# tj12323/GeoPurify

Measured on AMD Instinct MI355X. Metric: scenes/sec (ScanNet-val shape) + pooled-feature GB/s vs HBM peak, higher is better.
Workload: dtype f32 (student convolutions and pooling: f16 hi/lo split operands, 3 MFMAs per product, fp32 accumulate)

## Files before the change

geopurify_amd/csrc/sparse_conv_v2.hip:

```cpp
#include <cstring>
#include <type_traits>
#include <rocprim/device/device_scan.hpp>

#include <hip/hip_fp16.h>

#include <stdlib.h>

#include "gp_common.h"
#include "gp_gfx950.h"

namespace {

constexpr int TM = 256, TN = 256, TK = 32;
constexpr int NT2 = 512;
constexpr int APITCH = 32;
__device__ __forceinline__ int sw_slot(int row, int slot) {
    const int h = (0x78 >> (((row >> 2) & 3) * 2)) & 3;
    return slot ^ h;
}

__device__ __forceinline__ void pair_decode(int64_t i, int kv, const int32_t *__restrict__ R, int nchunks, int &c, int &k, int64_t &u) {
    const int row_q = (int)(i / kv);
    int lo = 0, hi = nchunks - 1;
    while (lo < hi) {
// ... 658 lines not shown
        continue;
    }
    for (int c = lane * 4; c < cout; c += 256) {
        float4 a = conv_gather_sum<GS_NL>(P, mypos, kv, cout, c, pair_base);
        float4 sc = scale ? *reinterpret_cast<const float4 *>(scale + c) : make_float4(1.f, 1.f, 1.f, 1.f);
        float4 sh = shift ? *reinterpret_cast<const float4 *>(shift + c) : make_float4(0.f, 0.f, 0.f, 0.f);
        a.x = a.x * sc.x + sh.x; a.y = a.y * sc.y + sh.y; a.z = a.z * sc.z + sh.z; a.w = a.w * sc.w + sh.w;
        if (residual) {
            float4 r = *reinterpret_cast<const float4 *>(residual + u * ld_res + c);
            a.x += r.x; a.y += r.y; a.z += r.z; a.w += r.w;
        }
        if (res_hi) {
            const _Float16 *rph = r_il ? res_hi + u * ld_rh + ((c >> 5) << 6) + (c & 31) : res_hi + u * ld_rh + c;
                    const _Float16 *rpl = r_il ? rph + 32 : res_lo + u * ld_rh + c;
                    const f16x4 rh = *reinterpret_cast<const f16x4 *>(rph), rl = *reinterpret_cast<const f16x4 *>(rpl);
            const float ri = res_inv ? res_inv[u] : 1.f;
            a.x += ((float)rh[0] + (float)rl[0]) * ri; a.y += ((float)rh[1] + (float)rl[1]) * ri;
            a.z += ((float)rh[2] + (float)rl[2]) * ri; a.w += ((float)rh[3] + (float)rl[3]) * ri;
        }
        if (relu) { a.x = fmaxf(a.x, 0.f); a.y = fmaxf(a.y, 0.f); a.z = fmaxf(a.z, 0.f); a.w = fmaxf(a.w, 0.f); }
        if (y) *reinterpret_cast<float4 *>(y + u * ld_y + c) = a;
        if (y_hi) {
            float v[4] = {a.x, a.y, a.z, a.w};
            f16x4 h, l;
            gp_split_f16<4>(v, h, l);
            _Float16 *ph = y_il ? y_hi + u * ld_yh + ((c >> 5) << 6) + (c & 31) : y_hi + u * ld_yh + c;
            _Float16 *pl = y_il ? ph + 32 : y_lo + u * ld_yh + c;
            *reinterpret_cast<f16x4 *>(ph) = h;
            *reinterpret_cast<f16x4 *>(pl) = l;
        }
    }
    }
}

template <int NL>
__device__ __forceinline__ void conv_gather_sum_q24(const unsigned char *__restrict__ pb, int64_t e_off, int mypos, int kv,
                                                    int cout, int c, bool act, int pair_base, float (&a)[8]) {
#pragma unroll
    for (int j = 0; j < 8; ++j) a[j] = 0.f;
    unsigned long long m = __ballot(mypos >= 0) & ((kv >= 64) ? ~0ull : ((1ull << kv) - 1ull));
    const int nq = cout >> 7;
    const unsigned char *pb_e = pb + e_off;
    while (m) {
        int kk[NL];
        u32x4 th[NL];
        u32x2 tl[NL];
        unsigned te[NL];
        int cntv = 0;
#pragma unroll
        for (int i = 0; i < NL; ++i) {
            if (m) { kk[i] = __builtin_ctzll(m); m &= m - 1; ++cntv; } else kk[i] = -1;
        }
#pragma unroll
        for (int i = 0; i < NL; ++i)
            if (i < cntv) {
                const unsigned pos = (unsigned)(__shfl(mypos, kk[i], 64) - pair_base);
                if (act) {
                    const unsigned o = (pos * (unsigned)cout + ((unsigned)c & ~127u)) * 3u, f = ((unsigned)c >> 3) & 15u;
                    th[i] = *reinterpret_cast<const u32x4 *>(pb + o + f * 16u);
                    tl[i] = *reinterpret_cast<const u32x2 *>(pb + o + 256u + f * 8u);
                    te[i] = pb_e[pos * (unsigned)nq + ((unsigned)c >> 7)];
                }
            }
#pragma unroll
        for (int i = 0; i < NL; ++i)
            if (i < cntv && act) {
                const float s = te[i] == 255u ? __uint_as_float(0x7fc00000u) : __uint_as_float((te[i] - 21u) << 23);
                const unsigned d[6] = {th[i][0], th[i][1], th[i][2], th[i][3], tl[i][0], tl[i][1]};
#pragma unroll
                for (int g = 0; g < 2; ++g) {
                    const unsigned u0 = __builtin_amdgcn_perm(0u, d[g * 3], 0x0c020100u);
                    const unsigned u1 = __builtin_amdgcn_perm(d[g * 3 + 1], d[g * 3], 0x0c050403u);
                    const unsigned u2 = __builtin_amdgcn_perm(d[g * 3 + 2], d[g * 3 + 1], 0x0c040302u);
                    const unsigned u3 = __builtin_amdgcn_perm(0u, d[g * 3 + 2], 0x0c030201u);
                    a[g * 4 + 0] = fmaf((float)u0 - 4194304.f, s, a[g * 4 + 0]);
                    a[g * 4 + 1] = fmaf((float)u1 - 4194304.f, s, a[g * 4 + 1]);
                    a[g * 4 + 2] = fmaf((float)u2 - 4194304.f, s, a[g * 4 + 2]);
                    a[g * 4 + 3] = fmaf((float)u3 - 4194304.f, s, a[g * 4 + 3]);
                }
            }
    }
}

template <bool WIDE , bool NO_CENTRE = false >
__global__ void __launch_bounds__(256) __attribute__((amdgpu_waves_per_eu(4, 4)))
conv_phase2_q24_kernel(const unsigned char *__restrict__ pb, int64_t e_off, const int32_t *__restrict__ pair_pos, int64_t nv,
                       int kv, int cout, const float *__restrict__ scale, const float *__restrict__ shift,
                       const float *__restrict__ residual, int64_t ld_res, int relu, float *__restrict__ y, int64_t ld_y,
                       _Float16 *__restrict__ y_hi, _Float16 *__restrict__ y_lo, int64_t ld_yh, int64_t row_begin, int64_t row_count,
                       int pair_base, float *__restrict__ y_inv_scale, const _Float16 *__restrict__ res_hi,
                       const _Float16 *__restrict__ res_lo, int64_t ld_rh, const float *__restrict__ res_inv, int plane_flags) {
    const bool y_il = (plane_flags & 2) != 0, r_il = (plane_flags & 4) != 0;
    const int lane = gp_lane();
    const int64_t wave0 = (blockIdx.x * (int64_t)blockDim.x + threadIdx.x) >> 6, n_waves = ((int64_t)gridDim.x * blockDim.x) >> 6;
    const int64_t row_end = (row_begin + row_count < nv) ? row_begin + row_count : nv;
    int64_t u = row_begin + wave0;
    if (u >= row_end) return;
    const bool rowscale = y_inv_scale && y_hi && cout <= 1024;
    const int kv_read = NO_CENTRE ? (kv >> 1) : -1;
    int mypos_next = (lane < kv && lane != kv_read) ? pair_pos[(int64_t)lane * nv + u] : -1;
    float sc0[8], sh0[8];
    {
        const int c = lane * 8;
#pragma unroll
        for (int h = 0; h < 2; ++h) {
            const float4 a = (scale && c < cout) ? *reinterpret_cast<const float4 *>(scale + c + h * 4) : make_float4(1.f, 1.f, 1.f, 1.f);
            const float4 b = (shift && c < cout) ? *reinterpret_cast<const float4 *>(shift + c + h * 4) : make_float4(0.f, 0.f, 0.f, 0.f);
            sc0[h * 4] = a.x; sc0[h * 4 + 1] = a.y; sc0[h * 4 + 2] = a.z; sc0[h * 4 + 3] = a.w;
            sh0[h * 4] = b.x; sh0[h * 4 + 1] = b.y; sh0[h * 4 + 2] = b.z; sh0[h * 4 + 3] = b.w;
        }
    }
    for (; u < row_end; u += n_waves) {
        const int mypos = mypos_next;
        if (u + n_waves < row_end) mypos_next = (lane < kv && lane != kv_read) ? pair_pos[(int64_t)lane * nv + u + n_waves] : -1;
        float av[WIDE ? 2 : 1][8];
        float amax = 0.f;
        auto block = [&](int c0, float (&a)[8]) {
            const int c = c0 + lane * 8;
            const bool act = c < cout;
            conv_gather_sum_q24<WIDE ? 4 : GS_NL>(pb, e_off, mypos, kv, cout, c, act, pair_base, a);
            if (!act) return;
            if (c0 == 0) {
#pragma unroll
                for (int j = 0; j < 8; ++j) a[j] = a[j] * sc0[j] + sh0[j];
            } else {
                float scv[8], shv[8];
#pragma unroll
                for (int h = 0; h < 2; ++h) {
                    const float4 sc = scale ? *reinterpret_cast<const float4 *>(scale + c + h * 4) : make_float4(1.f, 1.f, 1.f, 1.f);
                    const float4 sh = shift ? *reinterpret_cast<const float4 *>(shift + c + h * 4) : make_float4(0.f, 0.f, 0.f, 0.f);
                    scv[h * 4] = sc.x; scv[h * 4 + 1] = sc.y; scv[h * 4 + 2] = sc.z; scv[h * 4 + 3] = sc.w;
                    shv[h * 4] = sh.x; shv[h * 4 + 1] = sh.y; shv[h * 4 + 2] = sh.z; shv[h * 4 + 3] = sh.w;
                }
#pragma unroll
                for (int j = 0; j < 8; ++j) a[j] = a[j] * scv[j] + shv[j];
            }
            if (residual) {
                const float4 r0 = *reinterpret_cast<const float4 *>(residual + u * ld_res + c);
                const float4 r1 = *reinterpret_cast<const float4 *>(residual + u * ld_res + c + 4);
                a[0] += r0.x; a[1] += r0.y; a[2] += r0.z; a[3] += r0.w; a[4] += r1.x; a[5] += r1.y; a[6] += r1.z; a[7] += r1.w;
            }
            if (res_hi) {
                const _Float16 *rph = r_il ? res_hi + u * ld_rh + ((c >> 5) << 6) + (c & 31) : res_hi + u * ld_rh + c;
                const _Float16 *rpl = r_il ? rph + 32 : res_lo + u * ld_rh + c;
                const f16x8 rh = *reinterpret_cast<const f16x8 *>(rph), rl = *reinterpret_cast<const f16x8 *>(rpl);
                const float ri = res_inv ? res_inv[u] : 1.f;
#pragma unroll
                for (int j = 0; j < 8; ++j) a[j] += ((float)rh[j] + (float)rl[j]) * ri;
            }
            if (relu) {
#pragma unroll
                for (int j = 0; j < 8; ++j) a[j] = fmaxf(a[j], 0.f);
            }
            if (y) {
                *reinterpret_cast<float4 *>(y + u * ld_y + c) = make_float4(a[0], a[1], a[2], a[3]);
                *reinterpret_cast<float4 *>(y + u * ld_y + c + 4) = make_float4(a[4], a[5], a[6], a[7]);
            }
#pragma unroll
            for (int j = 0; j < 8; ++j) amax = fmaxf(amax, fabsf(a[j]));
        };
        auto split_store = [&](int c0, const float (&a)[8], float s) {
            const int c = c0 + lane * 8;
            if (c >= cout) return;
            f16x8 h, l;
#pragma unroll
            for (int j = 0; j < 8; ++j) gp_split_f16(a[j] * s, h, l, j);
            _Float16 *ph = y_il ? y_hi + u * ld_yh + ((c >> 5) << 6) + (c & 31) : y_hi + u * ld_yh + c;
            _Float16 *pl = y_il ? ph + 32 : y_lo + u * ld_yh + c;
            *reinterpret_cast<f16x8 *>(ph) = h;
            *reinterpret_cast<f16x8 *>(pl) = l;
        };
        block(0, av[0]);
        if (!rowscale && y_hi) split_store(0, av[0], 1.f);
        if constexpr (WIDE) {
            block(512, av[1]);
            if (!rowscale && y_hi) split_store(512, av[1], 1.f);
        }
        if (rowscale) {
            amax = gp_wave_max(amax);
            const float s = gp_pow2_for(amax);
            if (lane == 0) y_inv_scale[u] = 1.f / s;
            split_store(0, av[0], s);
            if constexpr (WIDE) split_store(512, av[1], s);
        } else if constexpr (WIDE) {
            for (int c0 = 1024; c0 < cout; c0 += 512) {
                block(c0, av[0]);
                if (y_hi) split_store(c0, av[0], 1.f);
            }
        }
    }
}

__global__ void split_rows_scaled_kernel(const float *__restrict__ x, int64_t ld_x, int d, int64_t n, _Float16 *__restrict__ hi,
// ... 151 lines not shown

extern "C" size_t gp_conv_chunk_plan_workspace_bytes(int64_t nv, int32_t granule_rows) {
    if (nv <= 0 || granule_rows <= 0) return 0;
    return (size_t)((nv + granule_rows - 1) / granule_rows) * 32 * sizeof(int32_t);
}
extern "C" int gp_conv_chunk_plan(const int32_t *nbr_map, int64_t nv, int32_t kv, int32_t granule_rows, int32_t col_tiles,
                                  int32_t target_tiles, int32_t max_chunks, int32_t *chunk_row_off, int32_t *n_chunks, void *workspace,
                                  size_t workspace_bytes, void *stream_) {
    GP_CHECK_ARG(nbr_map && chunk_row_off && n_chunks && workspace && nv > 0 && kv > 0 && kv <= 32, "gp_conv_chunk_plan: null/empty argument");
    GP_CHECK_ARG(granule_rows >= 64 && granule_rows <= 65535 && col_tiles >= 1 && target_tiles >= col_tiles && max_chunks >= 1, "gp_conv_chunk_plan: bad sizes");
    const int64_t ngran = (nv + granule_rows - 1) / granule_rows;
    GP_CHECK_ARG(workspace_bytes >= gp_conv_chunk_plan_workspace_bytes(nv, granule_rows), "gp_conv_chunk_plan: workspace too small");
    hipStream_t s = gp_stream(stream_);
    int32_t *cnt = static_cast<int32_t *>(workspace);
    chunk_count_kernel<<<dim3((unsigned)ngran, (unsigned)kv), 256, 0, s>>>(nbr_map, nv, kv, granule_rows, cnt);
    chunk_plan_kernel<<<1, 256, 0, s>>>(cnt, (int)ngran, kv, granule_rows, nv, col_tiles, target_tiles, max_chunks, chunk_row_off, n_chunks);
    GP_CHECK_LAUNCH();
    return GP_OK;
}

extern "C" int gp_conv_weights_split(const float *w, int32_t kv, int32_t cin, int32_t cout, float scale_pow2,
                                     void *w_hi, void *w_lo, void *stream_) {
    GP_CHECK_ARG(w && w_hi && w_lo && kv > 0 && cin > 0 && cout > 0, "gp_conv_weights_split: null/empty argument");
    weight_split_kernel<<<2048, 256, 0, gp_stream(stream_)>>>(w, kv, cin, cout, scale_pow2, static_cast<_Float16 *>(w_hi),
                                                              static_cast<_Float16 *>(w_lo));
    GP_CHECK_LAUNCH();
    return GP_OK;
}

extern "C" int gp_conv_weights_split_blocked(const float *w, int32_t kv, int32_t cin, int32_t cout, float scale_pow2, void *w_hi,
                                             void *w_lo, int32_t transpose_flip, void *stream_) {
    GP_CHECK_ARG(w && w_hi && w_lo && kv > 0 && cin > 0 && cout > 0, "gp_conv_weights_split_blocked: null/empty argument");
    GP_CHECK_ARG(cin % TK == 0 && cout % TN == 0, "gp_conv_weights_split_blocked: cin=%d must be a multiple of %d and cout=%d of %d", cin, TK, cout, TN);
    GP_CHECK_ARG(!transpose_flip || ((reinterpret_cast<uintptr_t>(w) & 15) == 0), "gp_conv_weights_split_blocked: w must be 16-byte aligned");
    weight_split_blocked_kernel<<<(unsigned)((int64_t)kv * (cout / TN) * (cin / TK)), 256, 0, gp_stream(stream_)>>>(
        w, kv, cin, cout, scale_pow2, static_cast<_Float16 *>(w_hi), static_cast<_Float16 *>(w_lo), transpose_flip);
    GP_CHECK_LAUNCH();
    return GP_OK;
}

extern "C" int gp_split_f16(const float *x, int64_t ld_x, int32_t d, int64_t n, void *hi, void *lo, int64_t ld_h,
                            void *stream_) {
    GP_CHECK_ARG(x && hi && lo && n > 0 && d > 0 && d % 4 == 0 && ld_x % 4 == 0 && ld_h % 4 == 0, "gp_split_f16: bad argument");
    split_rows_kernel<<<2048, 256, 0, gp_stream(stream_)>>>(x, ld_x, d, n, static_cast<_Float16 *>(hi), static_cast<_Float16 *>(lo), ld_h);
    GP_CHECK_LAUNCH();
    return GP_OK;
}

extern "C" int gp_pow2_scale(const float *x, int64_t ld_x, int32_t d, int64_t n, float *scale2, void *workspace,
                             size_t workspace_bytes, void *stream_) {
    GP_CHECK_ARG(x && scale2 && workspace && workspace_bytes >= 4 && n > 0 && d > 0 && d % 4 == 0 && ld_x % 4 == 0,
                 "gp_pow2_scale: bad argument");
    hipStream_t s = gp_stream(stream_);
    GP_CHECK_HIP(hipMemsetAsync(workspace, 0, 4, s));
    amax_kernel<<<1024, 256, 0, s>>>(x, ld_x, d, n, static_cast<unsigned *>(workspace));
    pow2_scale_kernel<<<1, 1, 0, s>>>(static_cast<const unsigned *>(workspace), scale2);
    GP_CHECK_LAUNCH();
    return GP_OK;
}

extern "C" int gp_split_f16_scaled(const float *x, int64_t ld_x, int32_t d, int64_t n, void *hi, void *lo, int64_t ld_h,
                                   const float *scale, float *row_inv_scale, const int32_t *dst_row, void *stream_) {
    GP_CHECK_ARG(x && hi && n > 0 && d > 0 && d % 4 == 0 && ld_x % 4 == 0 && ld_h % 4 == 0, "gp_split_f16_scaled: bad argument");
    GP_CHECK_ARG(lo || (d % 32 == 0 && ld_h >= 2 * (int64_t)d), "gp_split_f16_scaled: lo = NULL asks for interleaved rows in hi: d %% 32 == 0 and ld_h >= 2 d");
    GP_CHECK_ARG(!(scale && row_inv_scale), "gp_split_f16_scaled: one global scale OR per-row scales");
    int64_t waves = n < 16384 ? n : 16384;
    split_rows_scaled_kernel<<<(unsigned)((waves * 64 + 255) / 256), 256, 0, gp_stream(stream_)>>>(
        x, ld_x, d, n, static_cast<_Float16 *>(hi), static_cast<_Float16 *>(lo), ld_h, scale, row_inv_scale, dst_row);
    GP_CHECK_LAUNCH();
    return GP_OK;
}

extern "C" int gp_sparse_conv_f16x3(const float *x, int64_t ld_x, const void *x_hi, const void *x_lo, int64_t ld_xh,
                                    const int32_t *pair_in, const int32_t *pair_pos,
                                    const int32_t *pair_off, const int32_t *tile_start, const int32_t *tile_desc,
                                    int32_t nseg, int64_t num_pairs, int64_t nv, int32_t kv,
                                    const void *w_hi, const void *w_lo, int32_t cin, int32_t cout, float *partial,
                                    const float *scale, const float *shift, const float *residual, int64_t ld_res,
                                    int32_t relu, float *y, int64_t ld_y, void *y_hi, void *y_lo, int64_t ld_yh,
                                    int32_t num_chunks, const int32_t *chunk_row_off_host, const int32_t *chunk_tile_off_host,
                                    const int32_t *chunk_pair_off_host, const float *x_row_inv_scale, float *y_row_inv_scale,
                                    const void *res_hi, const void *res_lo, int64_t ld_rh, const float *res_row_inv_scale, int32_t w_blocked,
                                    int32_t plane_flags, void *stream_) {
    GP_CHECK_ARG(plane_flags >= 0 && plane_flags < 32, "gp_sparse_conv_f16x3: plane_flags is a mask of 1 (x interleaved), 2 (y interleaved), 4 (residual interleaved), 8 (fp32 partial rows), 16 (one dense offset: phase 1 writes y)");
    const bool direct = (plane_flags & 16) != 0;
    GP_CHECK_ARG(!direct || (kv == 1 && num_pairs == nv && x_hi && y && ld_y == cout && !scale && !shift && !residual && !res_hi && !relu && !y_hi &&
                             !y_row_inv_scale && !(g_gp_knobs[3] & 16)),
                 "gp_sparse_conv_f16x3: plane_flags bit 4 is for kv = 1 with a pair for every row, pre-split x, contiguous fp32 y and no epilogue");
    GP_CHECK_ARG(!(plane_flags & 1) || (x_hi && ld_xh % 64 == 0 && cin % 32 == 0), "gp_sparse_conv_f16x3: interleaved x rows come as ONE tensor (x_hi) of 2 x cin halfs per row");
    GP_CHECK_ARG(!(plane_flags & 2) || (y_hi && ld_yh % 64 == 0 && (uintptr_t)y_hi % 16 == 0), "gp_sparse_conv_f16x3: interleaved y rows go to ONE tensor (y_hi) of 2 x cout halfs per row");
    GP_CHECK_ARG(!(plane_flags & 4) || (res_hi && ld_rh % 64 == 0), "gp_sparse_conv_f16x3: interleaved residual rows come as ONE tensor (res_hi)");
    GP_CHECK_ARG(w_blocked == 0 || w_blocked == 1, "gp_sparse_conv_f16x3: w_blocked is 0 (row-major weights) or 1 (gp_conv_weights_split_blocked)");
    GP_CHECK_ARG(!res_hi || ((res_lo || (plane_flags & 4)) && !residual && ld_rh % 8 == 0 && (uintptr_t)res_hi % 16 == 0 && (uintptr_t)res_lo % 16 == 0),
                 "gp_sparse_conv_f16x3: the residual comes as fp32 rows OR as 16-byte aligned split planes (res_hi + res_lo), not both");
    GP_CHECK_ARG(res_hi || (!res_lo && !res_row_inv_scale), "gp_sparse_conv_f16x3: res_lo / res_row_inv_scale belong to res_hi");
    GP_CHECK_ARG((x || (x_hi && (x_lo || (plane_flags & 1)))) && pair_in && pair_pos && pair_off && tile_start && tile_desc && nseg > 0 && w_hi && w_lo && partial && (y || y_hi), "gp_sparse_conv_f16x3: null argument");
    GP_CHECK_ARG(!x_hi || (ld_xh % 8 == 0 && (uintptr_t)x_hi % 16 == 0 && (uintptr_t)x_lo % 16 == 0), "gp_sparse_conv_f16x3: pre-split rows must be 16-byte aligned");
    GP_CHECK_ARG(!(plane_flags & 1) || !(g_gp_knobs[3] & 16), "gp_sparse_conv_f16x3: interleaved x rows need the LDS-DMA path");
    GP_CHECK_ARG(!y_hi || ((y_lo || (plane_flags & 2)) && ld_yh % 4 == 0), "gp_sparse_conv_f16x3: y_hi/y_lo come as a pair");
    GP_CHECK_ARG(!x_row_inv_scale || x_hi, "gp_sparse_conv_f16x3: x_row_inv_scale belongs to pre-split operands (x_hi/x_lo)");
    GP_CHECK_ARG(!y_row_inv_scale || (y_hi && cout <= 1024), "gp_sparse_conv_f16x3: y_row_inv_scale needs y_hi/y_lo and cout <= 1024");
    GP_CHECK_ARG(nv > 0 && num_pairs > 0 && (kv == 27 || kv == 1), "gp_sparse_conv_f16x3: bad sizes");
    GP_CHECK_ARG(cin % TK == 0, "gp_sparse_conv_f16x3: cin=%d must be a multiple of %d", cin, TK);
    GP_CHECK_ARG(x_hi || (ld_x % 4 == 0 && (uintptr_t)x % 16 == 0), "gp_sparse_conv_f16x3: x rows must be 16-byte aligned");
    GP_SMEM_ATTR(conv_phase1_kernel<false>, sizeof(V2Smem));
    GP_SMEM_ATTR(conv_phase1_kernel<true>, sizeof(V2Smem));
    constexpr size_t P1_DMA_SMEM = sizeof(V2Smem) + TM * sizeof(float);
    GP_SMEM_ATTR(conv_phase1_dma_kernel, P1_DMA_SMEM);
    GP_SMEM_ATTR(conv_phase1_tuning_kernel, P1_DMA_SMEM);
    GP_SMEM_ATTR(conv_phase1_stamp_kernel, P1_DMA_SMEM);

    uint64_t *stamp = static_cast<uint64_t *>(g_gp_debug_ptr[1]);
    GP_CHECK_ARG(cout % TN == 0, "gp_sparse_conv_f16x3: cout=%d must be a multiple of %d on this path", cout, TN);
    hipStream_t s = gp_stream(stream_);
    int n_tiles = cout / TN;
    GP_CHECK_ARG((num_chunks >= 1) == (chunk_tile_off_host != nullptr) && (num_chunks >= 1) == (chunk_pair_off_host != nullptr) &&
                     (num_chunks >= 1) == (chunk_row_off_host != nullptr),
                 "gp_sparse_conv_f16x3: num_chunks=%d needs ALL THREE host chunk tables (row, tile and pair offsets), num_chunks=0 needs none",
                 num_chunks);
    if (num_chunks >= 1) {
        bool rows_ok = chunk_row_off_host[0] == 0 && chunk_row_off_host[num_chunks] == nv;
        for (int c = 0; c < num_chunks && rows_ok; ++c) rows_ok = chunk_row_off_host[c + 1] > chunk_row_off_host[c];
        GP_CHECK_ARG(rows_ok, "gp_sparse_conv_f16x3: the %d chunk row offsets do not cover rows 0 .. %lld in ascending order", num_chunks, (long long)nv);
    }
    const bool chunked = num_chunks >= 1;
    const int nchunk = chunked ? num_chunks : 1;
    constexpr int p2_wg_per_cu = 6;
    bool q24_fits = !(plane_flags & 8);
    for (int c = 0; c < nchunk; ++c) {
        const int64_t cp = chunked ? (int64_t)chunk_pair_off_host[c + 1] - chunk_pair_off_host[c] : num_pairs;
        if (cp * cout * 3 + 32 >= ((int64_t)1 << 32)) q24_fits = false;
    }
    for (int c = 0; c < nchunk; ++c) {
        int tile_begin = chunked ? chunk_tile_off_host[c] : 0;
        int tile_count = chunked ? chunk_tile_off_host[c + 1] - tile_begin : (int)(num_pairs / TM + nseg);
        int pair_base = chunked ? chunk_pair_off_host[c] : 0;
        int64_t row_begin = chunked ? chunk_row_off_host[c] : 0;
        int64_t row_count = chunked ? chunk_row_off_host[c + 1] - row_begin : nv;
        const int64_t chunk_pairs = chunked ? (int64_t)chunk_pair_off_host[c + 1] - pair_base : num_pairs;
        const int64_t q_e_off = (chunk_pairs * cout * 3 + 15) & ~(int64_t)15;
        const bool dma_path = x_hi && !(g_conv_ablate & 16);
        const bool q24 = dma_path && !(g_conv_ablate & 32) && q24_fits;
        if (tile_count > 0) {
            int64_t nblocks = (((int64_t)tile_count * n_tiles + 7) / 8) * 8;
            const int tune = (g_conv_ablate & ~16) | ((dma_path && (!q24_fits || direct)) ? 32 : 0);
#define P1_ARGS static_cast<const _Float16 *>(x_hi), static_cast<const _Float16 *>(x_lo), ld_xh, pair_in, pair_off, tile_start,              \
                reinterpret_cast<const int4 *>(tile_desc), nseg, kv, static_cast<const _Float16 *>(w_hi), static_cast<const _Float16 *>(w_lo), \
                cin, cout, direct ? y + (int64_t)pair_base * cout : partial, n_tiles, tune, tile_begin, tile_count, pair_base, x_row_inv_scale, stamp, \
                q_e_off, w_blocked, plane_flags & 1
            if (dma_path) {
                GP_CHECK_ARG(!stamp || g_gp_debug_bytes[1] >= (size_t)nblocks * 16 * sizeof(uint64_t),
                             "gp_sparse_conv_f16x3: the stamp buffer of gp_debug_ptr(1) holds %zu bytes, this launch writes %zu",
                             g_gp_debug_bytes[1], (size_t)nblocks * 16 * sizeof(uint64_t));
                if (stamp) conv_phase1_stamp_kernel<<<(unsigned)nblocks, NT2, P1_DMA_SMEM, s>>>(P1_ARGS);
                else if (tune) conv_phase1_tuning_kernel<<<(unsigned)nblocks, NT2, P1_DMA_SMEM, s>>>(P1_ARGS);
                else conv_phase1_dma_kernel<<<(unsigned)nblocks, NT2, P1_DMA_SMEM, s>>>(P1_ARGS);
            } else {
                GP_CHECK_ARG(x, "gp_sparse_conv_f16x3: fp32 x required for the register-staged path");
                GP_CHECK_ARG(!x_row_inv_scale, "gp_sparse_conv_f16x3: the register-staged path splits unscaled fp32 rows");
#define P1R_ARGS x, ld_x, pair_in, pair_off, tile_start, reinterpret_cast<const int4 *>(tile_desc), nseg, kv, static_cast<const _Float16 *>(w_hi), \
                 static_cast<const _Float16 *>(w_lo), cin, cout, partial, n_tiles, tune, tile_begin, tile_count, pair_base, w_blocked
                if (tune) conv_phase1_kernel<true><<<(unsigned)nblocks, NT2, sizeof(V2Smem), s>>>(P1R_ARGS);
                else conv_phase1_kernel<false><<<(unsigned)nblocks, NT2, sizeof(V2Smem), s>>>(P1R_ARGS);
#undef P1R_ARGS
            }
#undef P1_ARGS
        }
        if (direct) continue;
        const int64_t p2_full = (row_count * 64 + 255) / 256;
        int64_t p2_res = (int64_t)gp_cu_count() * p2_wg_per_cu;
        if (q24 && p2_wg_per_cu == 6) p2_res = (int64_t)gp_cu_count() * 4;
        const unsigned p2_grid = (unsigned)((p2_res > 0 && p2_res < p2_full) ? p2_res : p2_full);
#define P2Q_ARGS reinterpret_cast<const unsigned char *>(partial), q_e_off, pair_pos, nv, kv, cout, scale, shift, residual, ld_res, \
                 relu, y, ld_y, static_cast<_Float16 *>(y_hi), static_cast<_Float16 *>(y_lo), ld_yh, row_begin, row_count, pair_base, y_row_inv_scale, \
                 static_cast<const _Float16 *>(res_hi), static_cast<const _Float16 *>(res_lo), ld_rh, res_row_inv_scale, plane_flags
        if (q24 && cout <= 512 && (g_conv_ablate & 256)) conv_phase2_q24_kernel<false, true><<<p2_grid, 256, 0, s>>>(P2Q_ARGS);
        else if (q24 && cout > 512) conv_phase2_q24_kernel<true><<<p2_grid, 256, 0, s>>>(P2Q_ARGS);
        else if (q24) conv_phase2_q24_kernel<false><<<p2_grid, 256, 0, s>>>(P2Q_ARGS);
#undef P2Q_ARGS
        else
            conv_phase2_kernel<<<p2_grid, 256, 0, s>>>(
                partial, pair_pos, nv, kv, cout, scale, shift, residual, ld_res, relu, y, ld_y, static_cast<_Float16 *>(y_hi),
                static_cast<_Float16 *>(y_lo), ld_yh, row_begin, row_count, pair_base, y_row_inv_scale,
                static_cast<const _Float16 *>(res_hi), static_cast<const _Float16 *>(res_lo), ld_rh, res_row_inv_scale, plane_flags);
    }
    GP_CHECK_LAUNCH();
    return GP_OK;
}
```

geopurify_amd/ops.py:

```python
import ctypes

import numpy as np
import torch

from . import _lib
from ._lib import check


def _ptr(t):
    return ctypes.c_void_p(t.data_ptr()) if t is not None else None


def _stream():
    return ctypes.c_void_p(torch.cuda.current_stream().cuda_stream)


def _ws(nbytes, device):
    return torch.empty(max(int(nbytes), 256), dtype=torch.uint8, device=device)


def _chk(t, dtype, name):
    if t.dtype != dtype or not t.is_cuda or not t.is_contiguous():
        raise ValueError(f"{name}: expected contiguous CUDA {dtype}, got {t.dtype} cuda={t.is_cuda} contig={t.is_contiguous()}")
    return t
# ... 345 lines not shown
        if cout % 32 == 0 and cin % 256 == 0 and blocked is not False:
            hi = torch.empty((kv, cin // 256, cout // 32, 256, 32), dtype=torch.float16, device=w.device)
            lo = torch.empty_like(hi)
            check(lib.gp_conv_weights_split_blocked(_ptr(w), kv, cout, cin, float(scale_pow2), _ptr(hi), _ptr(lo), 1, _stream()),
                  "gp_conv_weights_split_blocked")
            return hi, lo
        return conv_weights_split(w.flip(0).transpose(1, 2).contiguous(), scale_pow2, blocked)
    if blocked is None:
        blocked = cin % 32 == 0 and cout % 256 == 0
    if blocked:
        hi = torch.empty((kv, cout // 256, cin // 32, 256, 32), dtype=torch.float16, device=w.device)
        lo = torch.empty_like(hi)
        check(lib.gp_conv_weights_split_blocked(_ptr(w), kv, cin, cout, float(scale_pow2), _ptr(hi), _ptr(lo), 0, _stream()),
              "gp_conv_weights_split_blocked")
        return hi, lo
    hi = torch.empty((kv, cout, cin), dtype=torch.float16, device=w.device)
    lo = torch.empty((kv, cout, cin), dtype=torch.float16, device=w.device)
    check(lib.gp_conv_weights_split(_ptr(w), kv, cin, cout, float(scale_pow2), _ptr(hi), _ptr(lo), _stream()),
          "gp_conv_weights_split")
    return hi, lo


def conv_weights_shape(w_hi):
    if w_hi.dim() == 5:
        return int(w_hi.shape[0]), int(w_hi.shape[1]) * 256, int(w_hi.shape[2]) * 32
    return tuple(int(v) for v in w_hi.shape)


def split_f16(x, d=None, scale=None, per_row=False, interleaved=False, dst_row=None, extra_zero_rows=0):
    lib = _lib.load()
    d = x.shape[1] if d is None else d
    if interleaved:
        assert per_row and d % 32 == 0, "interleaved rows are the row-scaled operand of the convolution"
        rows = torch.empty((x.shape[0], 2 * d), dtype=torch.float16, device=x.device)
        rinv = torch.empty(x.shape[0], dtype=torch.float32, device=x.device)
        check(lib.gp_split_f16_scaled(_ptr(x), x.stride(0), int(d), x.shape[0], _ptr(rows), None, rows.stride(0), None, _ptr(rinv),
                                      _ptr(dst_row), _stream()), "gp_split_f16_scaled")
        return rows, None, rinv
    hi = torch.empty((x.shape[0] + extra_zero_rows, d), dtype=torch.float16, device=x.device)
    lo = torch.empty((x.shape[0] + extra_zero_rows, d), dtype=torch.float16, device=x.device)
    if extra_zero_rows:
        hi[x.shape[0]:].zero_()
        lo[x.shape[0]:].zero_()
    if scale is None and not per_row:
        if dst_row is not None:
            raise ValueError("split_f16: dst_row needs a scaled form (scale= or per_row=True)")
        check(lib.gp_split_f16(_ptr(x), x.stride(0), int(d), x.shape[0], _ptr(hi), _ptr(lo), hi.stride(0), _stream()),
              "gp_split_f16")
        return hi, lo
    rinv = torch.empty(x.shape[0], dtype=torch.float32, device=x.device) if per_row else None
    check(lib.gp_split_f16_scaled(_ptr(x), x.stride(0), int(d), x.shape[0], _ptr(hi), _ptr(lo), hi.stride(0), _ptr(scale),
                                  _ptr(rinv), _ptr(dst_row), _stream()), "gp_split_f16_scaled")
    return (hi, lo, rinv) if per_row else (hi, lo)


def rcb_order(coords_sorted, chunk_rows=1024, leaf_rows=128):
    lib = _lib.load()
    _chk(coords_sorted, torch.int32, "coords")
    nv = coords_sorted.shape[0]
    sigma = torch.empty(nv, dtype=torch.int32, device=coords_sorted.device)
    rho = torch.empty(nv, dtype=torch.int32, device=coords_sorted.device)
    check(lib.gp_rcb_order(_ptr(coords_sorted), nv, int(chunk_rows), int(leaf_rows), _ptr(sigma), _ptr(rho), _stream()), "gp_rcb_order")
    return sigma, rho


def rows_renumber(nbr, sigma, rho):
    lib = _lib.load()
    nv, k = nbr.shape
    out = torch.empty_like(nbr)
    check(lib.gp_rows_renumber_i32(_ptr(nbr), nv, int(k), _ptr(sigma), _ptr(rho), _ptr(out), _stream()), "gp_rows_renumber_i32")
    return out


def pow2_scale(x, d=None):
    lib = _lib.load()
    d = x.shape[1] if d is None else d
    out = torch.empty(2, dtype=torch.float32, device=x.device)
    ws = _ws(256, x.device)
    check(lib.gp_pow2_scale(_ptr(x), x.stride(0), int(d), x.shape[0], _ptr(out), _ptr(ws), ws.numel(), _stream()), "gp_pow2_scale")
    return out


def sparse_conv_f16x3(x, pairs, w_hi, w_lo, scale=None, shift=None, residual=None, relu=False, out=None,
                      x_split=None, out_split=None, x_row_inv=None, out_row_inv=None, want_f32=True, fp32_partials=False, dense_single_offset=False):
    lib = _lib.load()
    res_planes = residual if isinstance(residual, (tuple, list)) else None
    if res_planes is not None:
        residual = None
    rh, rl, ri = (tuple(res_planes) + (None,))[:3] if res_planes is not None else (None, None, None)
    kv, cout, cin = conv_weights_shape(w_hi)
    w_blocked = int(w_hi.dim() == 5)
    nv = pairs.nv
    dev = w_hi.device
    if dense_single_offset:
        partial = torch.empty(64, dtype=torch.float32, device=dev)
    else:
        if pairs.partial is None or pairs.partial.shape[1] < cout or pairs.partial.shape[0] < max(pairs.max_chunk_pairs, 1):
            pairs.partial = torch.empty((max(pairs.max_chunk_pairs, 1), cout), dtype=torch.float32, device=dev)
        partial = pairs.partial
    if out is None and (want_f32 or out_split is None):
        out = torch.empty((nv, cout), dtype=torch.float32, device=dev)
    xh, xl = x_split if x_split is not None else (None, None)
    yh, yl = out_split if out_split is not None else (None, None)
    plane_flags = (1 if (xh is not None and xl is None) else 0) | (2 if (yh is not None and yl is None) else 0) | \
                  (4 if (rh is not None and rl is None) else 0) | (8 if fp32_partials else 0) | (16 if dense_single_offset else 0)
    check(lib.gp_sparse_conv_f16x3(_ptr(x), x.stride(0) if x is not None else 0, _ptr(xh), _ptr(xl),
                                   xh.stride(0) if xh is not None else 0, _ptr(pairs.pair_in), _ptr(pairs.pair_pos),
                                   _ptr(pairs.pair_off), _ptr(pairs.tile_start), _ptr(pairs.tile_desc), pairs.nseg, pairs.num_pairs, nv, kv, _ptr(w_hi), _ptr(w_lo), cin, cout,
                                   _ptr(partial), _ptr(scale), _ptr(shift), _ptr(residual),
                                   residual.stride(0) if residual is not None else 0, int(bool(relu)), _ptr(out),
                                   out.stride(0) if out is not None else 0, _ptr(yh), _ptr(yl), yh.stride(0) if yh is not None else 0,
                                   int(pairs.num_chunks), pairs.chunk_row_off, pairs.chunk_tile_off, pairs.chunk_pair_off,
                                   _ptr(x_row_inv), _ptr(out_row_inv), _ptr(rh), _ptr(rl), rh.stride(0) if rh is not None else 0, _ptr(ri),
                                   w_blocked, plane_flags, _stream()),
          "gp_sparse_conv_f16x3")
    return out


def interleave_planes(hi, lo):
    n, c = hi.shape
    return torch.stack([hi.reshape(n, c // 32, 32), lo.reshape(n, c // 32, 32)], dim=2).reshape(n, 2 * c).contiguous()


def deinterleave_planes(t):
    n, c2 = t.shape
    v = t.reshape(n, c2 // 64, 2, 32)
    return v[:, :, 0].reshape(n, c2 // 2).contiguous(), v[:, :, 1].reshape(n, c2 // 2).contiguous()


def l2norm_rows_(x, d=None):
    lib = _lib.load()
    d = x.shape[1] if d is None else d
    check(lib.gp_l2norm_rows(_ptr(x), x.stride(0), int(d), x.shape[0], _stream()), "gp_l2norm_rows")
    return x


def embed_head_f16x3(x_split, w_hi, w_lo, out_scale, x_row_inv=None, normalize=True, out=None, planes=False, want_f32=True, plane_rows=None):
    lib = _lib.load()
    hi, lo = x_split
    cout, cin = w_hi.shape[-2:]
    nv = hi.shape[0]
    _chk(hi, torch.float16, "x_hi"), _chk(lo, torch.float16, "x_lo")
    if hi.stride(0) != lo.stride(0) or hi.shape[1] < cin:
        raise ValueError("embed_head_f16x3: the hi / lo planes must share a row stride and hold cin channels")
    if out is None and (want_f32 or not planes):
        out = torch.empty((nv, cout), dtype=torch.float32, device=hi.device)
    eh = el = None
    if planes:
        eh = torch.empty((nv, cout), dtype=torch.float16, device=hi.device)
        el = torch.empty((nv, cout), dtype=torch.float16, device=hi.device)
    check(lib.gp_embed_head_f16x3(_ptr(hi), _ptr(lo), hi.stride(0), _ptr(x_row_inv), _ptr(w_hi), _ptr(w_lo), nv, int(cin), int(cout),
                                  float(out_scale), int(bool(normalize)), _ptr(out), out.stride(0) if out is not None else 0, _ptr(eh), _ptr(el),
                                  AFFINITY_PLANE_SCALE, _ptr(plane_rows) if planes else None, _stream()), "gp_embed_head_f16x3")
    return (out, (eh, el)) if planes else out


def knn_lattice(grid, coords_sorted, ids, k):
    lib = _lib.load()
    nv = coords_sorted.shape[0]
    dev = coords_sorted.device
    ws = _ws(lib.gp_knn_workspace_bytes(nv), dev)
    nbr = torch.empty((nv, k), dtype=torch.int32, device=dev)
    check(lib.gp_knn_lattice(_ptr(grid.buf), _ptr(coords_sorted), _ptr(ids), nv, int(k), _ptr(nbr), _ptr(ws),
                             ws.numel(), _stream()), "gp_knn_lattice")
    return nbr


def knn_batched(keys_sorted, ids, k, nbr=None, status=None, workspace=None):
    lib = _lib.load()
    _chk(keys_sorted, torch.int64, "keys")
    _chk(ids, torch.int32, "ids")
    nv, k = keys_sorted.shape[0], int(k)
    if keys_sorted.dim() != 1 or ids.shape != (nv,):
        raise ValueError(f"knn_batched: expected keys [nv] and ids [nv], got {list(keys_sorted.shape)} and {list(ids.shape)}")
    dev = keys_sorted.device
    if nbr is None:
        nbr = torch.empty((nv, max(k, 0)), dtype=torch.int32, device=dev)
    elif _chk(nbr, torch.int32, "nbr").shape != (nv, k):
        raise ValueError(f"knn_batched: expected nbr [{nv}, {k}], got {list(nbr.shape)}")
    if status is None:
        status = torch.empty(4, dtype=torch.int32, device=dev)
    elif _chk(status, torch.int32, "status").shape != (4,):
        raise ValueError(f"knn_batched: expected status [4], got {list(status.shape)}")
    ws = _ws(lib.gp_knn_batched_workspace_bytes(nv), dev) if workspace is None else _chk(workspace, torch.uint8, "workspace")
    check(lib.gp_knn_batched(_ptr(keys_sorted), _ptr(ids), nv, k, _ptr(nbr), _ptr(status), _ptr(ws), ws.numel(), _stream()),
          "gp_knn_batched")
    return nbr, status

# ... 911 lines not shown
```

Before: 45.39.

## Add software-pipelined row walk to q24 phase-2 gather for cout up to 512

```diff
diff --git a/geopurify_amd/csrc/sparse_conv_v2.hip b/geopurify_amd/csrc/sparse_conv_v2.hip
--- a/geopurify_amd/csrc/sparse_conv_v2.hip
+++ b/geopurify_amd/csrc/sparse_conv_v2.hip
@@ -764,8 +764,61 @@
     }
 }
 
-template <bool WIDE , bool NO_CENTRE = false >
-__global__ void __launch_bounds__(256) __attribute__((amdgpu_waves_per_eu(4, 4)))
+#ifndef GP_P2_NL
+#define GP_P2_NL 4
+#endif
+#ifndef GP_P2_WAVES
+#define GP_P2_WAVES 4
+#endif
+template <int NL, int NQ>
+__device__ __forceinline__ void q24_batch_issue(u32x4 (&th)[NL], u32x2 (&tl)[NL], unsigned (&te)[NL], unsigned (&tsel)[NL], int &cnt,
+                                                const unsigned char *__restrict__ pb, const unsigned char *__restrict__ pb_e, int mypos,
+                                                unsigned long long &m, unsigned off16, unsigned off8, bool act, int pair_base) {
+    const int left = __builtin_popcountll(m);
+    cnt = left < NL ? left : NL;
+#pragma unroll
+    for (int i = 0; i < NL; ++i)
+        if (i < cnt) {
+            const int k = __builtin_ctzll(m);
+            m &= m - 1;
+            const unsigned pos = (unsigned)(__builtin_amdgcn_readlane(mypos, k) - pair_base);
+            const unsigned char *row = pb + (size_t)(pos * (unsigned)(NQ * 384));
+            const unsigned eo = pos * (unsigned)NQ;
+            te[i] = *reinterpret_cast<const unsigned *>(pb_e + (size_t)(eo & ~3u));
+            tsel[i] = 0x0c0c0c00u | (eo & 3u);
+            if (act) {
+                th[i] = *reinterpret_cast<const u32x4 *>(row + off16);
+                tl[i] = *reinterpret_cast<const u32x2 *>(row + off8);
+            }
+        }
+}
+__device__ __forceinline__ void q24_row_decode(const u32x4 h, const u32x2 l, unsigned e, float (&a)[8]) {
+    const float s = e == 255u ? __uint_as_float(0x7fc00000u) : __uint_as_float((e - 21u) << 23);
+    const unsigned d0 = h.x, d1 = h.y, d2 = h.z, d3 = h.w, d4 = l.x, d5 = l.y;
+    const unsigned u0 = __builtin_amdgcn_perm(0u, d0, 0x0c020100u), u1 = __builtin_amdgcn_perm(d1, d0, 0x0c050403u);
+    const unsigned u2 = __builtin_amdgcn_perm(d2, d1, 0x0c040302u), u3 = __builtin_amdgcn_perm(0u, d2, 0x0c030201u);
+    const unsigned u4 = __builtin_amdgcn_perm(0u, d3, 0x0c020100u), u5 = __builtin_amdgcn_perm(d4, d3, 0x0c050403u);
+    const unsigned u6 = __builtin_amdgcn_perm(d5, d4, 0x0c040302u), u7 = __builtin_amdgcn_perm(0u, d5, 0x0c030201u);
+    a[0] = fmaf((float)u0 - 4194304.f, s, a[0]);
+    a[1] = fmaf((float)u1 - 4194304.f, s, a[1]);
+    a[2] = fmaf((float)u2 - 4194304.f, s, a[2]);
+    a[3] = fmaf((float)u3 - 4194304.f, s, a[3]);
+    a[4] = fmaf((float)u4 - 4194304.f, s, a[4]);
+    a[5] = fmaf((float)u5 - 4194304.f, s, a[5]);
+    a[6] = fmaf((float)u6 - 4194304.f, s, a[6]);
+    a[7] = fmaf((float)u7 - 4194304.f, s, a[7]);
+}
+template <int NL>
+__device__ __forceinline__ void q24_batch_decode(const u32x4 (&th)[NL], const u32x2 (&tl)[NL], const unsigned (&te)[NL], const unsigned (&tsel)[NL],
+                                                 int cnt, unsigned q, bool act, float (&a)[8]) {
+#pragma unroll
+    for (int i = 0; i < NL; ++i)
+        if (i < cnt && act) q24_row_decode(th[i], tl[i], __builtin_amdgcn_perm(0u, te[i], tsel[i] + q), a);
+}
+
+template <bool WIDE , bool NO_CENTRE = false ,
+          int WALK = 0 >
+__global__ void __launch_bounds__(256) __attribute__((amdgpu_waves_per_eu(WALK ? GP_P2_WAVES : 4, WALK ? GP_P2_WAVES : 4)))
 conv_phase2_q24_kernel(const unsigned char *__restrict__ pb, int64_t e_off, const int32_t *__restrict__ pair_pos, int64_t nv,
                        int kv, int cout, const float *__restrict__ scale, const float *__restrict__ shift,
                        const float *__restrict__ residual, int64_t ld_res, int relu, float *__restrict__ y, int64_t ld_y,
@@ -791,6 +844,106 @@
             sc0[h * 4] = a.x; sc0[h * 4 + 1] = a.y; sc0[h * 4 + 2] = a.z; sc0[h * 4 + 3] = a.w;
             sh0[h * 4] = b.x; sh0[h * 4 + 1] = b.y; sh0[h * 4 + 2] = b.z; sh0[h * 4 + 3] = b.w;
         }
+    }
+    if constexpr (WALK != 0) {
+        static_assert(!WIDE && !NO_CENTRE, "the pipelined walk is for cout = 256 and 512");
+        constexpr int NQ = 2 * WALK, NL = GP_P2_NL;
+        const int c = lane * 8;
+        const bool act = c < NQ * 128;
+        const unsigned q = (unsigned)c >> 7, f = ((unsigned)c >> 3) & 15u;
+        const unsigned off16 = q * 384u + f * 16u, off8 = q * 384u + 256u + f * 8u;
+        const unsigned char *pb_e = pb + e_off;
+        const unsigned long long kvmask = (kv >= 64) ? ~0ull : ((1ull << kv) - 1ull);
+        auto load_pos = [&](int64_t r) { return (lane < kv && r < row_end) ? pair_pos[(int64_t)lane * nv + r] : -1; };
+        auto wait_all = [] { __builtin_amdgcn_s_waitcnt(0x0f70); };
+        u32x4 thA[NL], thB[NL];
+        u32x2 tlA[NL], tlB[NL];
+        unsigned teA[NL], teB[NL], tselA[NL], tselB[NL];
+        int cntA, cntB;
+        int posA = mypos_next, posB = load_pos(u + n_waves);
+        unsigned long long mA = __ballot(posA >= 0) & kvmask;
+        q24_batch_issue<NL, NQ>(thA, tlA, teA, tselA, cntA, pb, pb_e, posA, mA, off16, off8, act, pair_base);
+        wait_all();
+        unsigned long long mB = __ballot(posB >= 0) & kvmask;
+        q24_batch_issue<NL, NQ>(thB, tlB, teB, tselB, cntB, pb, pb_e, posB, mB, off16, off8, act, pair_base);
+        int pos2 = load_pos(u + 2 * n_waves);
+        auto row = [&](u32x4 (&th)[NL], u32x2 (&tl)[NL], unsigned (&te)[NL], unsigned (&tsel)[NL], int &cnt, int &posX, unsigned long long &mX) __attribute__((always_inline)) {
+            u32x4 r0 = {0u, 0u, 0u, 0u}, r1 = {0u, 0u, 0u, 0u};
+            float ri = 1.f;
+            if (act) {
+                if (residual) {
+                    r0 = *reinterpret_cast<const u32x4 *>(residual + u * ld_res + c);
+                    r1 = *reinterpret_cast<const u32x4 *>(residual + u * ld_res + c + 4);
+                } else if (res_hi) {
+                    const _Float16 *rph = r_il ? res_hi + u * ld_rh + ((c >> 5) << 6) + (c & 31) : res_hi + u * ld_rh + c;
+                    const _Float16 *rpl = r_il ? rph + 32 : res_lo + u * ld_rh + c;
+                    r0 = *reinterpret_cast<const u32x4 *>(rph);
+                    r1 = *reinterpret_cast<const u32x4 *>(rpl);
+                    if (res_inv) ri = res_inv[u];
+                }
+            }
+            float a[8];
+#pragma unroll
+            for (int j = 0; j < 8; ++j) a[j] = 0.f;
+            q24_batch_decode<NL>(th, tl, te, tsel, cnt, q, act, a);
+            while (mX) {
+                q24_batch_issue<NL, NQ>(th, tl, te, tsel, cnt, pb, pb_e, posX, mX, off16, off8, act, pair_base);
+                q24_batch_decode<NL>(th, tl, te, tsel, cnt, q, act, a);
+            }
+            wait_all();
+            float amax = 0.f;
+            if (act) {
+#pragma unroll
+                for (int j = 0; j < 8; ++j) a[j] = a[j] * sc0[j] + sh0[j];
+                if (residual) {
+#pragma unroll
+                    for (int j = 0; j < 4; ++j) { a[j] += __uint_as_float(r0[j]); a[j + 4] += __uint_as_float(r1[j]); }
+                }
+                if (res_hi) {
+                    const f16x8 rh = __builtin_bit_cast(f16x8, r0), rl = __builtin_bit_cast(f16x8, r1);
+#pragma unroll
+                    for (int j = 0; j < 8; ++j) a[j] += ((float)rh[j] + (float)rl[j]) * ri;
+                }
+                if (relu) {
+#pragma unroll
+                    for (int j = 0; j < 8; ++j) a[j] = fmaxf(a[j], 0.f);
+                }
+                if (y) {
+                    *reinterpret_cast<float4 *>(y + u * ld_y + c) = make_float4(a[0], a[1], a[2], a[3]);
+                    *reinterpret_cast<float4 *>(y + u * ld_y + c + 4) = make_float4(a[4], a[5], a[6], a[7]);
+                }
+#pragma unroll
+                for (int j = 0; j < 8; ++j) amax = fmaxf(amax, fabsf(a[j]));
+            }
+            float s = 1.f;
+            if (rowscale) {
+                amax = gp_wave_max(amax);
+                s = gp_pow2_for(amax);
+                if (lane == 0) y_inv_scale[u] = 1.f / s;
+            }
+            if (y_hi && act) {
+                f16x8 h, l;
+#pragma unroll
+                for (int j = 0; j < 8; ++j) gp_split_f16(a[j] * s, h, l, j);
+                _Float16 *ph = y_il ? y_hi + u * ld_yh + ((c >> 5) << 6) + (c & 31) : y_hi + u * ld_yh + c;
+                _Float16 *pl = y_il ? ph + 32 : y_lo + u * ld_yh + c;
+                *reinterpret_cast<f16x8 *>(ph) = h;
+                *reinterpret_cast<f16x8 *>(pl) = l;
+            }
+            posX = pos2;
+            mX = __ballot(posX >= 0) & kvmask;
+            q24_batch_issue<NL, NQ>(th, tl, te, tsel, cnt, pb, pb_e, posX, mX, off16, off8, act, pair_base);
+            pos2 = load_pos(u + 3 * n_waves);
+        };
+        for (;;) {
+            row(thA, tlA, teA, tselA, cntA, posA, mA);
+            u += n_waves;
+            if (u >= row_end) break;
+            row(thB, tlB, teB, tselB, cntB, posB, mB);
+            u += n_waves;
+            if (u >= row_end) break;
+        }
+        return;
     }
     for (; u < row_end; u += n_waves) {
         const int mypos = mypos_next;
@@ -1108,7 +1261,7 @@
                                     const int32_t *chunk_pair_off_host, const float *x_row_inv_scale, float *y_row_inv_scale,
                                     const void *res_hi, const void *res_lo, int64_t ld_rh, const float *res_row_inv_scale, int32_t w_blocked,
                                     int32_t plane_flags, void *stream_) {
-    GP_CHECK_ARG(plane_flags >= 0 && plane_flags < 32, "gp_sparse_conv_f16x3: plane_flags is a mask of 1 (x interleaved), 2 (y interleaved), 4 (residual interleaved), 8 (fp32 partial rows), 16 (one dense offset: phase 1 writes y)");
+    GP_CHECK_ARG(plane_flags >= 0 && plane_flags < 64, "gp_sparse_conv_f16x3: plane_flags is a mask of 1 (x interleaved), 2 (y interleaved), 4 (residual interleaved), 8 (fp32 partial rows), 16 (one dense offset: phase 1 writes y), 32 (phase 2 walks one row at a time)");
     const bool direct = (plane_flags & 16) != 0;
     GP_CHECK_ARG(!direct || (kv == 1 && num_pairs == nv && x_hi && y && ld_y == cout && !scale && !shift && !residual && !res_hi && !relu && !y_hi &&
                              !y_row_inv_scale && !(g_gp_knobs[3] & 16)),
@@ -1196,11 +1349,15 @@
         const int64_t p2_full = (row_count * 64 + 255) / 256;
         int64_t p2_res = (int64_t)gp_cu_count() * p2_wg_per_cu;
         if (q24 && p2_wg_per_cu == 6) p2_res = (int64_t)gp_cu_count() * 4;
+        const bool p2_pipe = q24 && cout <= 512 && !(plane_flags & 32) && !(g_conv_ablate & 256);
+        if (p2_pipe) p2_res = (int64_t)gp_cu_count() * GP_P2_WAVES;
         const unsigned p2_grid = (unsigned)((p2_res > 0 && p2_res < p2_full) ? p2_res : p2_full);
 #define P2Q_ARGS reinterpret_cast<const unsigned char *>(partial), q_e_off, pair_pos, nv, kv, cout, scale, shift, residual, ld_res, \
                  relu, y, ld_y, static_cast<_Float16 *>(y_hi), static_cast<_Float16 *>(y_lo), ld_yh, row_begin, row_count, pair_base, y_row_inv_scale, \
                  static_cast<const _Float16 *>(res_hi), static_cast<const _Float16 *>(res_lo), ld_rh, res_row_inv_scale, plane_flags
-        if (q24 && cout <= 512 && (g_conv_ablate & 256)) conv_phase2_q24_kernel<false, true><<<p2_grid, 256, 0, s>>>(P2Q_ARGS);
+        if (p2_pipe && cout == 512) conv_phase2_q24_kernel<false, false, 2><<<p2_grid, 256, 0, s>>>(P2Q_ARGS);
+        else if (p2_pipe) conv_phase2_q24_kernel<false, false, 1><<<p2_grid, 256, 0, s>>>(P2Q_ARGS);
+        else if (q24 && cout <= 512 && (g_conv_ablate & 256)) conv_phase2_q24_kernel<false, true><<<p2_grid, 256, 0, s>>>(P2Q_ARGS);
         else if (q24 && cout > 512) conv_phase2_q24_kernel<true><<<p2_grid, 256, 0, s>>>(P2Q_ARGS);
         else if (q24) conv_phase2_q24_kernel<false><<<p2_grid, 256, 0, s>>>(P2Q_ARGS);
 #undef P2Q_ARGS
diff --git a/geopurify_amd/ops.py b/geopurify_amd/ops.py
--- a/geopurify_amd/ops.py
+++ b/geopurify_amd/ops.py
@@ -451,7 +451,8 @@
 
 
 def sparse_conv_f16x3(x, pairs, w_hi, w_lo, scale=None, shift=None, residual=None, relu=False, out=None,
-                      x_split=None, out_split=None, x_row_inv=None, out_row_inv=None, want_f32=True, fp32_partials=False, dense_single_offset=False):
+                      x_split=None, out_split=None, x_row_inv=None, out_row_inv=None, want_f32=True, fp32_partials=False, dense_single_offset=False,
+                      reference_walk=False):
     lib = _lib.load()
     res_planes = residual if isinstance(residual, (tuple, list)) else None
     if res_planes is not None:
@@ -472,7 +473,7 @@
     xh, xl = x_split if x_split is not None else (None, None)
     yh, yl = out_split if out_split is not None else (None, None)
     plane_flags = (1 if (xh is not None and xl is None) else 0) | (2 if (yh is not None and yl is None) else 0) | \
-                  (4 if (rh is not None and rl is None) else 0) | (8 if fp32_partials else 0) | (16 if dense_single_offset else 0)
+                  (4 if (rh is not None and rl is None) else 0) | (8 if fp32_partials else 0) | (16 if dense_single_offset else 0) | (32 if reference_walk else 0)
     check(lib.gp_sparse_conv_f16x3(_ptr(x), x.stride(0) if x is not None else 0, _ptr(xh), _ptr(xl),
                                    xh.stride(0) if xh is not None else 0, _ptr(pairs.pair_in), _ptr(pairs.pair_pos),
                                    _ptr(pairs.pair_off), _ptr(pairs.tile_start), _ptr(pairs.tile_desc), pairs.nseg, pairs.num_pairs, nv, kv, _ptr(w_hi), _ptr(w_lo), cin, cout,
```

After: 46.05, median of 6. 1.01x the previous value.
